# fabianschenk/REVO

Hardware: AMD Instinct MI355X
Metric: tracked frames/sec at 640x480, 4-level pyramid; ATE vs reference (higher is better)
Workload: dtype f32

## Files before the change

### revo_amd/csrc/revo_dev.h

```cpp
#pragma once
#include <hip/hip_runtime.h>
#include <stdint.h>
#include "../../include/revo_hip.h"

#define REVO_L REVO_MAX_LEVELS

struct LevelGeom {
  int w, h;
  int npix;
  float fx, fy, cx, cy;
  int patch;
  int hist_w, hist_h;
  int nchunk;
  int chunk_rows;
  int wpr;
  int nms_block_base;
  int has_orig;
  int pix_base;
  int edt_rows;
  int edt_block_base;
  int strip_base;
  int cc_base;
  int band_rows, nbands, band_base;
};

struct PyrGeom {
  int frame0;
  int fstride;
  int n_levels;
  int total_nms_blocks, total_pix, total_edt_blocks, total_strips, total_cc;
  int total_bands, any_banded;
  int hyst_force;
  int hyst_heavy_runs;
  int total_tiles;
  int pts_staged;
  float depth_min, depth_max;
  int canny_low, canny_high;
  int use_edge_hist;
  float n_percentage;
  double fill_thr[REVO_L];
  LevelGeom lv[REVO_L];
};

struct FramePlanes {
  uint8_t* gray[REVO_L];
  float* depth[REVO_L];
  uint2* cs[REVO_L];
  uint8_t* edges[REVO_L];
  uint8_t* edges_orig[REVO_L];
  int* scratch[REVO_L];
  float4* pts[REVO_L];
  float4* pts_trk[REVO_L];
  float* dt[REVO_L];
  float4* table[REVO_L];
  uint8_t* hist[REVO_L];
  int* chunk[REVO_L];
  unsigned* cmask[REVO_L];
  uint8_t* vb[REVO_L];
  int* npts;
  int* hist_nz;
  int* strip_tot;
  uint32_t* ebits[REVO_L];
  int* need_full;
  int* hyst_heavy;
  int* tile_base;
  float* stage[REVO_L];
  unsigned short* epre[REVO_L];
  int* stage_base;
};

struct PairDesc {
  const float4* pts[REVO_L];
  const int* npts;
  const float* dt[REVO_L];
  float R[9];
  float T[3];
};

struct TrackParams {
  int pyr_min_lvl, pyr_max_lvl;
  int lvl_begin, lvl_end;
  int check_init;
  int eval_only;
  int kspec[REVO_L];
  int redundant_n;
  float lambda_success_fac, lambda_fail_fac;
  float lambda_initial[REVO_L], step_size_min[REVO_L], convergence_eps[REVO_L];
  int max_its[REVO_L];
  float edge_distance[REVO_L];
  float huber_edge;
  int use_edge_filter;
  struct { float fx, fy, cx, cy; int w, h; } cam[REVO_L];
  int exact_sums;
};

struct EvalOut {
  float A[36];
  float b[6];
  float error;
  float mean_err;
  float sum_w, sum_u;
  int good, bad;
};

#define REVO_MAX_WIDTH 2048
#define NMS_ROWS 6
#define EDT_ROW_PX 1280
#ifndef REVO_HYST_LDS_MAX
#define REVO_HYST_LDS_MAX 158720
#endif
#ifndef TRACK_THREADS
#define TRACK_THREADS 512
#endif
#ifndef TRACK_MAX_CLUSTER
#define TRACK_MAX_CLUSTER 32
#endif
#define TRACK_KMAX 4
#define TRACK_NVAL 48
#define TRACK_NVAL_X 132
#define TRACK_MAIL_NVAL TRACK_NVAL_X

void launch_gray_depth(const PyrGeom& g, const FramePlanes& p, const uint8_t* d_bgr, const float* d_depth_f32,
                       const uint16_t* d_depth_u16, float u16_alpha, int B, hipStream_t s);
void launch_pyrdown(const PyrGeom& g, const FramePlanes& p, int lvl, int B, hipStream_t s, int parts = 3, bool stage_edges = false);
void launch_edge_prefix(const PyrGeom& g, const FramePlanes& p, int B, hipStream_t s);
void launch_canny_nms(const PyrGeom& g, const FramePlanes& p, int B, hipStream_t s);
void launch_hyst(const PyrGeom& g, const FramePlanes& p, int B, hipStream_t s);
void launch_fill(const PyrGeom& g, const FramePlanes& p, int B, hipStream_t s);
void launch_compact(const PyrGeom& g, const FramePlanes& p, int B, hipStream_t s);
void launch_tile_points(const PyrGeom& g, const FramePlanes& p, int B, hipStream_t s, int which = 3);
void launch_pyrdown_bgr(const uint8_t* src, int w, int h, uint8_t* dst, hipStream_t s);
void launch_colored_pcl(const PyrGeom& g, const FramePlanes& p, int frame, int lvl, int dense, const uint8_t* bgr_lvl,
                        int* chunk, unsigned* cmask, int* total, int cap, float* out8, hipStream_t s);
void launch_keyframe(const PyrGeom& g, const FramePlanes& p, int f0, int fstride, int count, hipStream_t s, int which = 3);
int launch_track(const PairDesc* d_descs, const TrackParams& prm, revo_pair_result* d_out, EvalOut* d_eval,
                 int n_pairs, unsigned long long* d_mail, unsigned* epoch_io, int cluster, unsigned* d_resident, hipStream_t s);
void launch_track_gate(unsigned* d_resident, unsigned want, hipStream_t s);
int launch_track_one(const PairDesc& desc, const TrackParams& prm, revo_pair_result* out, EvalOut* eval_out,
                     unsigned long long* d_mail, unsigned* epoch_io, int cluster, unsigned* seq_ptr, unsigned seq_val,
                     unsigned* d_resident, hipStream_t s);
void launch_solve6(const float* d_Ab , int n, float* d_x , hipStream_t s);
int track_blocks_per_cu();
void launch_grad_table(const PyrGeom& g, const FramePlanes& p, int f0, int fstride, int count, hipStream_t s);
struct VoteArgs { float RT[3][12]; const float4* pts[3]; const int* n[3]; };
void launch_vote(const PyrGeom& g, const FramePlanes& curr, int curr_frame, int lvl, int n_clouds, const VoteArgs& va,
                 int* d_marks , int* d_hist8 , unsigned* d_done ,
                 int* h_out8 , unsigned seq_val, int use_orig_edges,
                 hipStream_t s);
void launch_copy_cloud(float4* dst, const float4* src, int* dst_n, const int* src_n, hipStream_t s);
struct VoteDesc {
  float RT[3][12]; const float4* pts[3]; const int* n[3]; int n_clouds;
  const uint8_t* edges; const float* depth;
  int* marks; int* hist8; unsigned* done;
  int* host_out;
};
struct CloudCopyDesc { float4* dst; const float4* src; int* dst_n; const int* src_n; };
struct CopySeg { const void* src; void* dst; size_t bytes; };
void launch_vote_multi(const PyrGeom& g, int lvl, int n, const VoteDesc* d_descs, unsigned seq_val, hipStream_t s);
void launch_copy_cloud_multi(int n, const CloudCopyDesc* d_descs, hipStream_t s);
void launch_copy_segments(int n, const CopySeg* d_segs, hipStream_t s);

#define INFO_THREADS 256
#define INFO_CHUNK 1024
#define INFO_MAX_GROUPS 32
#define INFO_PART_DOUBLES 64
struct InfoParams {
  float fx, fy, cx, cy;
  int w, h;
  float edge_distance, huber_edge;
  int use_edge_filter, level;
};
static inline int info_groups(int npix) {
  const int g = (npix + 8 * INFO_CHUNK - 1) / (8 * INFO_CHUNK);
  return g < 1 ? 1 : (g > INFO_MAX_GROUPS ? INFO_MAX_GROUPS : g);
}
void launch_pair_info(const PairDesc* d_descs, const void* d_pose, int pose_stride, int flag_word, const InfoParams& prm,
                      int n_pairs, double* d_part, int* d_cnt, unsigned* d_ticket, revo_pair_info* d_out, hipStream_t s);
```

### revo_amd/csrc/revo_pyramid.hip

```cpp
#include "revo_dev.h"
#include "revo_nms_px.h"
#include <type_traits>

namespace {

#ifdef REVO_BUILD_PRIO
#define BUILD_PRIO() __builtin_amdgcn_s_setprio(REVO_BUILD_PRIO)
#else
#define BUILD_PRIO()
#endif

__device__ __forceinline__ int level_of(const PyrGeom& g, int v, int LevelGeom::*base) {
  int l = 0;
#pragma unroll
  for (int k = 1; k < REVO_L; ++k)
    if (k < g.n_levels && v >= g.lv[k].*base) l = k;
  return l;
}
__device__ __forceinline__ int clampi(int v, int lo, int hi) { return v < lo ? lo : (v > hi ? hi : v); }
__device__ __forceinline__ int reflect101(int i, int n) {
  if (i < 0) i = -i;
  if (i >= n) i = 2 * n - 2 - i;
  return i;
}

__device__ __forceinline__ uint32_t gray4(uint32_t a, uint32_t b, uint32_t c) {
  const int B0 = a & 255, G0 = (a >> 8) & 255, R0 = (a >> 16) & 255, B1 = a >> 24;
  const int G1 = b & 255, R1 = (b >> 8) & 255, B2 = (b >> 16) & 255, G2 = b >> 24;
  const int R2 = c & 255, B3 = (c >> 8) & 255, G3 = (c >> 16) & 255, R3 = c >> 24;
  const uint32_t y0 = (uint32_t)(B0 * 1868 + G0 * 9617 + R0 * 4899 + 8192) >> 14;
  const uint32_t y1 = (uint32_t)(B1 * 1868 + G1 * 9617 + R1 * 4899 + 8192) >> 14;
  const uint32_t y2 = (uint32_t)(B2 * 1868 + G2 * 9617 + R2 * 4899 + 8192) >> 14;
  const uint32_t y3 = (uint32_t)(B3 * 1868 + G3 * 9617 + R3 * 4899 + 8192) >> 14;
  return y0 | (y1 << 8) | (y2 << 16) | (y3 << 24);
}
__global__ void __launch_bounds__(256) k_gray_depth(const uint8_t* __restrict__ bgr, const float* __restrict__ depth_f32,
                                                    const uint16_t* __restrict__ depth_u16, float alpha,
                                                    uint8_t* __restrict__ gray, float* __restrict__ depth_out, int npix, int frame0) {
  BUILD_PRIO();
  const int f = frame0 + blockIdx.z;
  const int g16 = blockIdx.x * 256 + threadIdx.x;
  if (g16 * 16 >= npix) return;
  const uint4* src = reinterpret_cast<const uint4*>(bgr + (size_t)f * npix * 3) + (size_t)g16 * 3;
  const uint4 p = src[0], q = src[1], r = src[2];
  reinterpret_cast<uint4*>(gray + (size_t)f * npix)[g16] =
      make_uint4(gray4(p.x, p.y, p.z), gray4(p.w, q.x, q.y), gray4(q.z, q.w, r.x), gray4(r.y, r.z, r.w));
  if (depth_out == depth_f32) return;
  float4* dst = reinterpret_cast<float4*>(depth_out + (size_t)f * npix) + (size_t)g16 * 4;
  if (depth_u16) {
    const uint4* raw = reinterpret_cast<const uint4*>(depth_u16 + (size_t)f * npix) + (size_t)g16 * 2;
    const uint4 u = raw[0], v = raw[1];
    const uint32_t wds[8] = {u.x, u.y, u.z, u.w, v.x, v.y, v.z, v.w};
#pragma unroll
    for (int k = 0; k < 4; ++k) {
      float4 d;
      d.x = (float)(wds[2 * k] & 0xffff) * alpha + 0.0f;
      d.y = (float)(wds[2 * k] >> 16) * alpha + 0.0f;
      d.z = (float)(wds[2 * k + 1] & 0xffff) * alpha + 0.0f;
      d.w = (float)(wds[2 * k + 1] >> 16) * alpha + 0.0f;
      dst[k] = d;
    }
  } else {
    const float4* in = reinterpret_cast<const float4*>(depth_f32 + (size_t)f * npix) + (size_t)g16 * 4;
    const float4 d0 = in[0], d1 = in[1], d2 = in[2], d3 = in[3];
    dst[0] = d0; dst[1] = d1; dst[2] = d2; dst[3] = d3;
  }
}

struct EdgeStage {
  const uint2* cs;
  const unsigned short* epre;
  const int* base;
  float* out;
  int wpr, tiles_total;
};
template <bool GRAY, bool DEPTH, bool STAGE = false>
__global__ void __launch_bounds__(256) k_pyrdown(const uint8_t* __restrict__ src, int sw, int sh, uint8_t* __restrict__ dst,
                                                 int dw, int dh, const float* __restrict__ dsrc, float* __restrict__ ddst, int frame0,
                                                 int fstride, uint8_t* __restrict__ vsrc, float dmin, float dmax, EdgeStage es) {
  BUILD_PRIO();
  static_assert(!STAGE || DEPTH, "staging rides on the depth half");
  const int f = frame0 + fstride * blockIdx.z;
  src += (size_t)f * sw * sh;
  dst += (size_t)f * dw * dh;
  dsrc += (size_t)f * sw * sh;
  ddst += (size_t)f * dw * dh;
  vsrc += (size_t)f * (sw >> 3) * sh;
  const int gw = dw >> 2, gh = (dh + 1) >> 1;
  const int i = blockIdx.x * 256 + threadIdx.x;
  if (i >= gw * gh) return;
  const int gx = i % gw, gy = i / gw;
  const int oy = 2 * gy;
  const int nrows = (oy + 1 < dh) ? 2 : 1;
  const int swords = sw >> 2;
  const uint32_t* srcw = reinterpret_cast<const uint32_t*>(src);
  const int w1i = 2 * gx;
  int hs[7][4];
#pragma unroll
  for (int r = 0; r < 7; ++r) {
    if (GRAY && r < 2 * nrows + 3) {
      const uint32_t* row = srcw + (size_t)reflect101(2 * oy - 2 + r, sh) * swords;
      uint32_t w0 = row[max(w1i - 1, 0)];
      const uint32_t w1 = row[w1i], w2 = row[w1i + 1];
      uint32_t w3 = row[min(w1i + 2, swords - 1)];
      if (gx == 0) w0 = (((w1 >> 16) & 0xffu) << 16) | (((w1 >> 8) & 0xffu) << 24);
      if (gx == gw - 1) w3 = (w2 >> 16) & 0xffu;
      const int b[11] = {(int)((w0 >> 16) & 0xffu), (int)(w0 >> 24),
                         (int)(w1 & 0xffu), (int)((w1 >> 8) & 0xffu), (int)((w1 >> 16) & 0xffu), (int)(w1 >> 24),
                         (int)(w2 & 0xffu), (int)((w2 >> 8) & 0xffu), (int)((w2 >> 16) & 0xffu), (int)(w2 >> 24),
                         (int)(w3 & 0xffu)};
#pragma unroll
      for (int j = 0; j < 4; ++j) hs[r][j] = b[2 * j] + b[2 * j + 4] + 4 * (b[2 * j + 1] + b[2 * j + 3]) + 6 * b[2 * j + 2];
    } else {
#pragma unroll
      for (int j = 0; j < 4; ++j) hs[r][j] = 0;
    }
  }
#pragma unroll
  for (int q = 0; q < 2; ++q) {
    if (q >= nrows) break;
    if (GRAY) {
      uint32_t packed = 0;
#pragma unroll
      for (int j = 0; j < 4; ++j) {
        const int v = hs[2 * q][j] + hs[2 * q + 4][j] + 4 * (hs[2 * q + 1][j] + hs[2 * q + 3][j]) + 6 * hs[2 * q + 2][j];
        packed |= (uint32_t)((v + 128) >> 8) << (8 * j);
      }
      reinterpret_cast<uint32_t*>(dst + (size_t)(oy + q) * dw)[gx] = packed;
    }
    if (!DEPTH) continue;
    const float* d0 = dsrc + (size_t)(2 * (oy + q)) * sw + 8 * gx;
    const float4 a0 = *reinterpret_cast<const float4*>(d0), a1 = *reinterpret_cast<const float4*>(d0 + 4);
    const float4 c0 = *reinterpret_cast<const float4*>(d0 + sw), c1 = *reinterpret_cast<const float4*>(d0 + sw + 4);
    const float top[8] = {a0.x, a0.y, a0.z, a0.w, a1.x, a1.y, a1.z, a1.w};
    const float bot[8] = {c0.x, c0.y, c0.z, c0.w, c1.x, c1.y, c1.z, c1.w};
    unsigned vt = 0, vbm = 0;
#pragma unroll
    for (int k = 0; k < 8; ++k) {
      vt |= (isfinite(top[k]) && top[k] > dmin && top[k] < dmax) ? 1u << k : 0u;
      vbm |= (isfinite(bot[k]) && bot[k] > dmin && bot[k] < dmax) ? 1u << k : 0u;
    }
    vsrc[(size_t)(2 * (oy + q)) * (sw >> 3) + gx] = (uint8_t)vt;
    vsrc[(size_t)(2 * (oy + q) + 1) * (sw >> 3) + gx] = (uint8_t)vbm;
    if (STAGE) {
      const int wc = (8 * gx) >> 5, sh8 = (8 * gx) & 31;
#pragma unroll
      for (int rr = 0; rr < 2; ++rr) {
        const int y = 2 * (oy + q) + rr;
        const uint32_t E = es.cs[((size_t)f * sh + y) * es.wpr + wc].y;
        uint32_t eb = (E >> sh8) & 0xffu;
        if (eb) {
          const int tile = (y >> 5) * es.wpr + wc;
          int pos = es.base[(size_t)f * es.tiles_total + tile] + (int)es.epre[((size_t)f * sh + y) * es.wpr + wc] +
                    __popc(E & ((1u << sh8) - 1u));
// ... 1385 lines not shown
  const uint32_t E = y < h ? csw[(size_t)y * wpr + wc].y : 0u;
  uint32_t v = (has_vb && y < h) ? tile_valid_word(g, pl, l, f, y, wc, E) : E;
  if (!has_vb)
    for (uint32_t m = v; m; m &= m - 1) {
      const int b = __ffs(m) - 1;
      if (!depth_ok(depth[(size_t)y * w + x0 + b], g.depth_min, g.depth_max)) v &= ~(1u << b);
    }
  const int cnt = __popc(v);
  int incl = cnt;
#pragma unroll
  for (int o = 1; o < 32; o <<= 1) {
    const int u = __shfl_up(incl, o, 32);
    if (r >= o) incl += u;
  }
  const int total = __shfl(incl, 31, 32);
  if (total == 0) return;
  unsigned short* src = s_src[threadIdx.x >> 5];
  const bool staged = STAGED && has_vb;
  unsigned short* esrc = s_esrc[STAGED ? (threadIdx.x >> 5) : 0];
  {
    int o = incl - cnt;
    int ebase = 0;
    if (staged) {
      const int ec = __popc(E);
      int ei = ec;
#pragma unroll
      for (int q = 1; q < 32; q <<= 1) {
        const int u = __shfl_up(ei, q, 32);
        if (r >= q) ei += u;
      }
      ebase = ei - ec;
    }
    for (uint32_t m = v; m; m &= m - 1, ++o) {
      const int b = __ffs(m) - 1;
      src[o] = (unsigned short)((r << 5) | b);
      if (staged) esrc[o] = (unsigned short)(ebase + __popc(E & ((1u << b) - 1u)));
    }
  }
  float4* out = pl.pts_trk[l] + (size_t)f * lv.npix + tile_first;
  const float* stage_t = staged ? pl.stage[l] + (size_t)f * lv.npix + pl.stage_base[(size_t)f * g.total_tiles + tg] : nullptr;
  for (int k0 = r; k0 < total; k0 += 4 * 32) {
    int rb[4];
    float Z[4];
#pragma unroll
    for (int q = 0; q < 4; ++q) rb[q] = k0 + 32 * q < total ? (int)src[k0 + 32 * q] : -1;
    if (staged) {
#pragma unroll
      for (int q = 0; q < 4; ++q) Z[q] = rb[q] >= 0 ? stage_t[esrc[k0 + 32 * q]] : 0.0f;
    } else {
#pragma unroll
      for (int q = 0; q < 4; ++q) Z[q] = rb[q] >= 0 ? depth[(size_t)(y0 + (rb[q] >> 5)) * w + x0 + (rb[q] & 31)] : 0.0f;
    }
#pragma unroll
    for (int q = 0; q < 4; ++q) {
      if (rb[q] < 0) continue;
      const float X = __fdiv_rn(Z[q] * ((float)(x0 + (rb[q] & 31)) - lv.cx), lv.fx);
      const float Y = __fdiv_rn(Z[q] * ((float)(y0 + (rb[q] >> 5)) - lv.cy), lv.fy);
      out[k0 + 32 * q] = make_float4(X, Y, Z[q], 1.0f);
    }
  }
}

__device__ __forceinline__ int block_exclusive_scan(int* a, int n, int* s_part) {
  const int tid = threadIdx.x, lane = tid & 63, wave = tid >> 6;
  const int per = (n + 1023) / 1024;
  const int b = min(n, tid * per), e = min(n, b + per);
  int sum = 0;
  for (int i = b; i < e; ++i) sum += a[i];
  int incl = sum;
#pragma unroll
  for (int o = 1; o < 64; o <<= 1) {
    const int v = __shfl_up(incl, o);
    if (lane >= o) incl += v;
  }
  if (lane == 63) s_part[wave] = incl;
  __syncthreads();
  int run = incl - sum, total = 0;
#pragma unroll
  for (int k = 0; k < 16; ++k) {
    const int wv = s_part[k];
    run += k < wave ? wv : 0;
    total += wv;
  }
  for (int i = b; i < e; ++i) { const int c = a[i]; a[i] = run; run += c; }
  return total;
}


__global__ void __launch_bounds__(256) k_pyrdown_bgr(const uint8_t* __restrict__ src, int w, int h,
                                                     uint8_t* __restrict__ dst) {
  const int dw = w >> 1, dh = h >> 1;
  const int i = blockIdx.x * 256 + threadIdx.x;
  if (i >= dw * dh) return;
  const int x = i % dw, y = i / dw;
  const int kk[5] = {1, 4, 6, 4, 1};
  int acc[3] = {0, 0, 0};
#pragma unroll
  for (int j = 0; j < 5; ++j) {
    const uint8_t* row = src + (size_t)reflect101(2 * y + j - 2, h) * w * 3;
    int rs[3] = {0, 0, 0};
#pragma unroll
    for (int t = 0; t < 5; ++t) {
      const uint8_t* px = row + (size_t)reflect101(2 * x + t - 2, w) * 3;
      rs[0] += kk[t] * px[0]; rs[1] += kk[t] * px[1]; rs[2] += kk[t] * px[2];
    }
    acc[0] += kk[j] * rs[0]; acc[1] += kk[j] * rs[1]; acc[2] += kk[j] * rs[2];
  }
  uint8_t* o = dst + (size_t)i * 3;
  o[0] = (uint8_t)((acc[0] + 128) >> 8); o[1] = (uint8_t)((acc[1] + 128) >> 8); o[2] = (uint8_t)((acc[2] + 128) >> 8);
}

template <bool WRITE>
__global__ void __launch_bounds__(256) k_pcl_walk(LevelGeom lv, float dmin, float dmax, const float* __restrict__ depth,
                                                  const uint8_t* __restrict__ edges, const uint8_t* __restrict__ bgr,
                                                  int dense, int* __restrict__ chunk, unsigned* __restrict__ cmask,
                                                  const int* __restrict__ total, int cap, float4* __restrict__ out) {
  const int i = blockIdx.x * 256 + threadIdx.x;
  if (i >= lv.w * lv.nchunk) return;
  const int x = i % lv.w, c = i / lv.w;
  const int yb = c * lv.chunk_rows, ye = min(lv.h, yb + lv.chunk_rows);
  const size_t slot = (size_t)x * lv.nchunk + c;
  if (!WRITE) {
    unsigned vm = 0;
    for (int y = yb; y < ye; ++y) {
      const size_t p = (size_t)y * lv.w + x;
      if ((dense || edges[p]) && depth_ok(depth[p], dmin, dmax)) vm |= 1u << (y - yb);
    }
    cmask[slot] = vm;
    chunk[slot] = __popc(vm);
  } else {
    if (*total > cap) return;
    int o = chunk[slot];
    for (unsigned m = cmask[slot]; m; m &= m - 1) {
      const int y = yb + __ffs(m) - 1;
      const size_t p = (size_t)y * lv.w + x;
      const float Z = depth[p];
      const float X = __fdiv_rn(Z * ((float)x - lv.cx), lv.fx);
      const float Y = __fdiv_rn(Z * ((float)y - lv.cy), lv.fy);
      const uint8_t* px = bgr + p * 3;
      out[2 * o] = make_float4(X, Y, Z, 1.0f);
      out[2 * o + 1] = make_float4(__fdiv_rn((float)px[2], 255.0f), __fdiv_rn((float)px[1], 255.0f),
                                   __fdiv_rn((float)px[0], 255.0f), 1.0f);
      ++o;
    }
  }
}

__global__ void __launch_bounds__(1024) k_pcl_scan(int* chunk, int n, int* total) {
  __shared__ int s_part[1024];
  const int t = block_exclusive_scan(chunk, n, s_part);
  if (threadIdx.x == 0) *total = t;
}

#define EDT_INF (1 << 29)
#define EDT_THREADS 1024
#define EDT_COL_GROUPS(h) ((h) > 1024 ? 64 : ((h) > 512 ? 32 : 16))
__global__ void __launch_bounds__(EDT_THREADS) k_edt_cols(PyrGeom g, FramePlanes pl, int f0, int fstride, int nframes) {
  __shared__ int s_first[EDT_THREADS];
  __shared__ int s_last[EDT_THREADS];
  const int f = f0 + (blockIdx.x % nframes) * fstride;
  int l = 0, sidx = blockIdx.x / nframes, ngroups = 16, ncols = 64;
  for (int k = 0; k < g.n_levels; ++k) {
    ngroups = EDT_COL_GROUPS(g.lv[k].h);
    ncols = EDT_THREADS / ngroups;
    const int ns = (g.lv[k].w + ncols - 1) / ncols;
    if (sidx < ns) { l = k; break; }
    sidx -= ns;
  }
  const LevelGeom& lv = g.lv[l];
  const int col = threadIdx.x % ncols, grp = threadIdx.x / ncols;
  const int x = sidx * ncols + col;
  const int rpg = (lv.h + ngroups - 1) / ngroups;
  const int yb = min(lv.h, grp * rpg), ye = min(lv.h, yb + rpg);
  const bool in = x < lv.w;
  const uint8_t* edges = pl.edges[l] + (size_t)f * lv.npix;
  unsigned em = 0;
  if ((lv.w & 31) == 0 && (ncols & 31) == 0) {
    const uint2* csw = pl.cs[l] + (size_t)f * lv.h * lv.wpr;
    const int r = threadIdx.x & 31;
    const int wc = (sidx * ncols + (col & ~31)) >> 5;
    uint32_t v = 0;
    if (yb + r < ye && wc < lv.wpr) v = csw[(size_t)(yb + r) * lv.wpr + wc].y;
    em = tile_transpose32(v, r);
    if (!in) em = 0;
  } else if (in) {
#pragma unroll 8
    for (int y = yb; y < ye; ++y) em |= (edges[(size_t)y * lv.w + x] ? 1u : 0u) << (y - yb);
  }
  s_first[grp * ncols + col] = em ? yb + __ffs(em) - 1 : EDT_INF;
  s_last[grp * ncols + col] = em ? yb + 31 - __clz(em) : -EDT_INF;
  __syncthreads();
  if (!in) return;
  int above = -EDT_INF, below = EDT_INF;
  for (int k = 0; k < grp; ++k) above = max(above, s_last[k * ncols + col]);
  for (int k = ngroups - 1; k > grp; --k) below = min(below, s_first[k * ncols + col]);
  uint16_t* gd = reinterpret_cast<uint16_t*>(pl.scratch[l]) + (size_t)f * lv.npix;
  const int FAR = 1 << 20;
  int du = (above <= -EDT_INF) ? FAR : (yb - above);
  const int dbelow = (below >= EDT_INF) ? FAR : (below - yb);
  for (int y = yb; y < ye; ++y) {
    const int k = y - yb;
    const unsigned hi = em >> k;
    du = (hi & 1u) ? 0 : du;
    const int dn = hi ? __ffs(hi) - 1 : dbelow - k;
    const int m = min(du, dn);
    gd[(size_t)y * lv.w + x] = (uint16_t)(m >= 0xffff ? 0xffff : m);
    du += 1;
  }
}

__device__ __forceinline__ float sqrt_rn_int(float x) {
  const float s = __builtin_amdgcn_sqrtf(x);
  const unsigned si = __float_as_uint(s);
  const float sd = __uint_as_float(si - 1u), su = __uint_as_float(si + 1u);
  const float rd = __builtin_fmaf(-sd, s, x), ru = __builtin_fmaf(-su, s, x);
  float r = (rd <= 0.0f) ? sd : s;
  r = (ru > 0.0f) ? su : r;
  return r;
}
__global__ void __launch_bounds__(256) k_edt_rows(PyrGeom g, FramePlanes pl, int f0, int fstride) {
  extern __shared__ int s_g2[];
  const int f = f0 + blockIdx.z * fstride;
  const int l = level_of(g, blockIdx.x, &LevelGeom::edt_block_base);
  const LevelGeom lv = g.lv[l];
  const int w = lv.w;
  const int y0 = (blockIdx.x - lv.edt_block_base) * lv.edt_rows;
  const int nr = min(lv.edt_rows, lv.h - y0);
  const int pad = w + 4, pitch = w + 2 * pad;
  const uint16_t* gd = reinterpret_cast<const uint16_t*>(pl.scratch[l]) + (size_t)f * lv.npix + (size_t)y0 * w;
  const int4 inf4 = make_int4(EDT_INF, EDT_INF, EDT_INF, EDT_INF);
  const int padq = pad >> 2, wq = w >> 2;
  for (int r = 0; r < nr; ++r) {
    int4* row4 = reinterpret_cast<int4*>(s_g2 + r * pitch);
    for (int i = threadIdx.x; i < padq; i += 256) { row4[i] = inf4; row4[padq + wq + i] = inf4; }
    const uint2* src = reinterpret_cast<const uint2*>(gd + r * w);
    for (int i = threadIdx.x; i < wq; i += 256) {
      const uint2 q = src[i];
      const int d0 = (int)(q.x & 0xffffu), d1 = (int)(q.x >> 16), d2 = (int)(q.y & 0xffffu), d3 = (int)(q.y >> 16);
      row4[padq + i] = make_int4(d0 == 0xffff ? EDT_INF : __mul24(d0, d0), d1 == 0xffff ? EDT_INF : __mul24(d1, d1),
                                 d2 == 0xffff ? EDT_INF : __mul24(d2, d2), d3 == 0xffff ? EDT_INF : __mul24(d3, d3));
    }
  }
  __syncthreads();
  float* dt = pl.dt[l] + (size_t)f * lv.npix + (size_t)y0 * w;
  const int dq = 256 / w, dr = 256 - dq * w;
  int r = threadIdx.x / w, x = threadIdx.x - r * w;
  for (int p = threadIdx.x; p < nr * w; p += 256) {
    const int* c = s_g2 + r * pitch + pad + x;
    int best = c[0];
    for (int d = 1; d < w && d * d < best; d += 4) {
      int m = best;
#pragma unroll
      for (int j = 0; j < 4; ++j) {
        const int dj = d + j;
        m = min(m, dj * dj + min(c[-dj], c[dj]));
      }
      best = m;
    }
    dt[p] = best >= EDT_INF ? sqrtf(1e15f) : sqrt_rn_int((float)best);
    x += dr; r += dq;
    if (x >= w) { x -= w; ++r; }
  }
}

__global__ void __launch_bounds__(256) k_grad_table(PyrGeom g, FramePlanes pl, int f0, int fstride) {
  const int f = f0 + blockIdx.z * fstride;
  const int l = blockIdx.y;
  const LevelGeom& lv = g.lv[l];
  const int i = blockIdx.x * 256 + threadIdx.x;
  if (i >= lv.npix) return;
  const float* dt = pl.dt[l] + (size_t)f * lv.npix;
  float4 o = make_float4(0.f, 0.f, 0.f, 0.f);
  if (i >= lv.w && i < lv.w * (lv.h - 1)) {
    o.x = 0.5f * (dt[i - 1] - dt[i + 1]);
    o.y = 0.5f * (dt[i - lv.w] - dt[i + lv.w]);
    o.z = dt[i];
  }
  pl.table[l][(size_t)f * lv.npix + i] = o;
}

__global__ void __launch_bounds__(256) k_vote_mark(VoteArgs a, float fx, float fy, float cx, float cy, int W, int H,
                                                   int* marks) {
  const int c = blockIdx.y;
  const int n = *a.n[c];
  const float* R = a.RT[c];
  const float* T = R + 9;
  const float4* pts = a.pts[c];
  for (int i = blockIdx.x * 256 + threadIdx.x; i < n; i += gridDim.x * 256) {
    const float4 p = pts[i];
    float q[3];
#pragma unroll
    for (int r = 0; r < 3; ++r) q[r] = ((R[r] * p.x + R[3 + r] * p.y) + R[6 + r] * p.z) + T[r];
    const float u = __fdiv_rn(fx * q[0], q[2]) + cx;
    const float v = __fdiv_rn(fy * q[1], q[2]) + cy;
    if (u >= 0 && u < (float)W && v >= 0 && v < (float)H)
      atomicOr(&marks[(int)floorf(v) * W + (int)floorf(u)], 1 << c);
  }
}

__global__ void __launch_bounds__(256) k_vote_hist(int* marks, const uint8_t* edges, const float* depth, int npix,
                                                   float dmin, float dmax, int* hist8, unsigned* done, int* host_out,
                                                   unsigned seq_val) {
  __shared__ int s_h[8];
  __shared__ bool s_last;
  if (threadIdx.x < 8) s_h[threadIdx.x] = 0;
  __syncthreads();
  for (int i = blockIdx.x * 256 + threadIdx.x; i < npix; i += gridDim.x * 256) {
    const int m = marks[i];
    if (m) marks[i] = 0;
    const float Z = depth[i];
    if (depth_ok(Z, dmin, dmax)) {
      const int val = __popc(m);
      atomicAdd(&s_h[val], 1);
      if (edges[i] > 0) atomicAdd(&s_h[4 + val], 1);
    }
  }
  __syncthreads();
  if (threadIdx.x < 8 && s_h[threadIdx.x]) atomicAdd(&hist8[threadIdx.x], s_h[threadIdx.x]);
  __threadfence();
  __syncthreads();
  if (threadIdx.x == 0) s_last = (atomicAdd(done, 1u) == gridDim.x - 1);
  __syncthreads();
  if (s_last) {
    if (threadIdx.x < 8) host_out[threadIdx.x] = atomicExch(&hist8[threadIdx.x], 0);
    if (threadIdx.x == 0) *done = 0u;
    __threadfence_system();
    __syncthreads();
    if (threadIdx.x == 0) *(volatile int*)&host_out[8] = (int)seq_val;
  }
}

__global__ void __launch_bounds__(256) k_copy_cloud(float4* __restrict__ dst, const float4* __restrict__ src,
                                                    int* __restrict__ dst_n, const int* __restrict__ src_n) {
  const int n = *src_n;
  for (int i = blockIdx.x * 256 + threadIdx.x; i < n; i += gridDim.x * 256) dst[i] = src[i];
  if (blockIdx.x == 0 && threadIdx.x == 0) *dst_n = n;
}

__global__ void __launch_bounds__(256) k_vote_mark_multi(const VoteDesc* __restrict__ descs, float fx, float fy, float cx,
                                                         float cy, int W, int H) {
  const VoteDesc& d = descs[blockIdx.z];
  const int c = blockIdx.y;
  if (c >= d.n_clouds) return;
  const int n = *d.n[c];
  const float* R = d.RT[c];
  const float* T = R + 9;
  const float4* pts = d.pts[c];
  int* marks = d.marks;
  for (int i = blockIdx.x * 256 + threadIdx.x; i < n; i += gridDim.x * 256) {
    const float4 p = pts[i];
    float q[3];
#pragma unroll
    for (int r = 0; r < 3; ++r) q[r] = ((R[r] * p.x + R[3 + r] * p.y) + R[6 + r] * p.z) + T[r];
    const float u = __fdiv_rn(fx * q[0], q[2]) + cx;
    const float v = __fdiv_rn(fy * q[1], q[2]) + cy;
    if (u >= 0 && u < (float)W && v >= 0 && v < (float)H)
      atomicOr(&marks[(int)floorf(v) * W + (int)floorf(u)], 1 << c);
  }
}

__global__ void __launch_bounds__(256) k_vote_hist_multi(const VoteDesc* __restrict__ descs, int npix, float dmin, float dmax,
                                                         unsigned seq_val) {
  const VoteDesc& d = descs[blockIdx.y];
  int* marks = d.marks;
  __shared__ int s_h[8];
  __shared__ bool s_last;
  if (threadIdx.x < 8) s_h[threadIdx.x] = 0;
  __syncthreads();
  for (int i = blockIdx.x * 256 + threadIdx.x; i < npix; i += gridDim.x * 256) {
    const int m = marks[i];
    if (m) marks[i] = 0;
    const float Z = d.depth[i];
    if (depth_ok(Z, dmin, dmax)) {
      const int val = __popc(m);
      atomicAdd(&s_h[val], 1);
      if (d.edges[i] > 0) atomicAdd(&s_h[4 + val], 1);
    }
  }
  __syncthreads();
  if (threadIdx.x < 8 && s_h[threadIdx.x]) atomicAdd(&d.hist8[threadIdx.x], s_h[threadIdx.x]);
  __threadfence();
  __syncthreads();
  if (threadIdx.x == 0) s_last = (atomicAdd(d.done, 1u) == gridDim.x - 1);
  __syncthreads();
  if (s_last) {
    if (threadIdx.x < 8) d.host_out[threadIdx.x] = atomicExch(&d.hist8[threadIdx.x], 0);
    if (threadIdx.x == 0) *d.done = 0u;
    __threadfence_system();
    __syncthreads();
    if (threadIdx.x == 0) *(volatile int*)&d.host_out[8] = (int)seq_val;
  }
}

__global__ void __launch_bounds__(256) k_copy_cloud_multi(const CloudCopyDesc* __restrict__ descs) {
  const CloudCopyDesc& d = descs[blockIdx.y];
  const int n = *d.src_n;
  for (int i = blockIdx.x * 256 + threadIdx.x; i < n; i += gridDim.x * 256) d.dst[i] = d.src[i];
  if (blockIdx.x == 0 && threadIdx.x == 0) *d.dst_n = n;
}

__global__ void __launch_bounds__(256) k_copy_segments(const CopySeg* __restrict__ segs) {
  const CopySeg& sg = segs[blockIdx.y];
  const char* src = (const char*)sg.src;
  char* dst = (char*)sg.dst;
  const size_t bytes = sg.bytes;
  const size_t step = (size_t)gridDim.x * 256;
  if ((((uintptr_t)src | (uintptr_t)dst | bytes) & 15) == 0) {
    const uint4* s4 = (const uint4*)src;
    uint4* d4 = (uint4*)dst;
    for (size_t i = blockIdx.x * 256 + threadIdx.x; i < bytes / 16; i += step) d4[i] = s4[i];
  } else {
    for (size_t i = blockIdx.x * 256 + threadIdx.x; i < bytes; i += step) dst[i] = src[i];
  }
}
// ... 7 lines not shown
  hipLaunchKernelGGL(k_gray_depth, grid, dim3(256), 0, s, d_bgr, d_depth_f32, d_depth_u16, u16_alpha, p.gray[0],
                     p.depth[0], npix, g.frame0);
}

void launch_pyrdown(const PyrGeom& g, const FramePlanes& p, int lvl, int B, hipStream_t s, int parts, bool stage_edges) {
  const LevelGeom& d = g.lv[lvl];
  const LevelGeom& sl = g.lv[lvl - 1];
  dim3 grid(((d.w / 4) * ((d.h + 1) / 2) + 255) / 256, 1, B);
  EdgeStage es{};
  if (stage_edges) {
    int tb = 0;
    for (int k = 0; k < lvl - 1; ++k) tb += g.lv[k].wpr * g.lv[k].nchunk;
    es.cs = p.cs[lvl - 1]; es.epre = p.epre[lvl - 1]; es.base = p.stage_base + tb; es.out = p.stage[lvl - 1];
    es.wpr = sl.wpr; es.tiles_total = g.total_tiles;
  }
#define PYRDOWN_ARGS p.gray[lvl - 1], sl.w, sl.h, p.gray[lvl], d.w, d.h, p.depth[lvl - 1], p.depth[lvl], g.frame0, g.fstride, p.vb[lvl - 1], g.depth_min, g.depth_max, es
  if (parts == 1) hipLaunchKernelGGL((k_pyrdown<true, false>), grid, dim3(256), 0, s, PYRDOWN_ARGS);
  else if (parts == 2 && stage_edges) hipLaunchKernelGGL((k_pyrdown<false, true, true>), grid, dim3(256), 0, s, PYRDOWN_ARGS);
  else if (parts == 2) hipLaunchKernelGGL((k_pyrdown<false, true>), grid, dim3(256), 0, s, PYRDOWN_ARGS);
  else hipLaunchKernelGGL((k_pyrdown<true, true>), grid, dim3(256), 0, s, PYRDOWN_ARGS);
#undef PYRDOWN_ARGS
}

void launch_edge_prefix(const PyrGeom& g, const FramePlanes& p, int B, hipStream_t s) {
  if (g.n_levels < 2) return;
  hipLaunchKernelGGL(k_edge_prefix, dim3((g.n_levels - 1) * B), dim3(1024), 0, s, g, p);
}

void launch_canny_nms(const PyrGeom& g, const FramePlanes& p, int B, hipStream_t s) {
  hipLaunchKernelGGL(k_canny_nms4, dim3(g.total_nms_blocks, 1, B), dim3(256), 0, s, g, p);
}

void launch_hyst(const PyrGeom& g, const FramePlanes& p, int B, hipStream_t s) {
  size_t e_bytes = 0, ec_bytes = 0;
  for (int l = 0; l < g.n_levels; ++l) {
    const size_t nw = (size_t)g.lv[l].h * g.lv[l].wpr;
    const size_t e = ((size_t)(g.lv[l].h + 2) * g.lv[l].wpr + 2) * 4, c = (nw + (nw + 2) / 2) * 4;
    e_bytes = e > e_bytes ? e : e_bytes;
    ec_bytes = e + c > ec_bytes ? e + c : ec_bytes;
  }
  static bool attr_set = false;
  if (!attr_set) {
    (void)hipFuncSetAttribute(reinterpret_cast<const void*>(k_hyst<true>), hipFuncAttributeMaxDynamicSharedMemorySize, REVO_HYST_LDS_MAX);
    (void)hipFuncSetAttribute(reinterpret_cast<const void*>(k_hyst<false>), hipFuncAttributeMaxDynamicSharedMemorySize, REVO_HYST_LDS_MAX);
    attr_set = true;
  }
  const int force = g.hyst_force;
  const bool fits_single = ec_bytes + 4096 <= REVO_HYST_LDS_MAX;
  const bool banded = force >= 0 ? force == 1 : !fits_single;
  const int only_flagged = banded && g.total_bands > 0 ? 1 : 0;
  if (only_flagged) {
    static bool attr2 = false;
    if (!attr2) {
      (void)hipFuncSetAttribute(reinterpret_cast<const void*>(k_hyst_band), hipFuncAttributeMaxDynamicSharedMemorySize, HB_LDS_WORDS * 4);
      (void)hipFuncSetAttribute(reinterpret_cast<const void*>(k_hyst_out), hipFuncAttributeMaxDynamicSharedMemorySize, HB_LDS_WORDS * 4);
      (void)hipFuncSetAttribute(reinterpret_cast<const void*>(k_hyst_seam), hipFuncAttributeMaxDynamicSharedMemorySize, 64 * 1024);
      (void)hipGetLastError();
      attr2 = true;
    }
    size_t seam_lds = 4, out_lds = 4;
    for (int l = 0; l < g.n_levels; ++l) {
      const LevelGeom& lv = g.lv[l];
      const size_t nwb = (size_t)lv.band_rows * lv.wpr;
      out_lds = std::max(out_lds, nwb * 4);
      if (lv.nbands > 1) seam_lds = std::max(seam_lds, (size_t)lv.nbands * (size_t)(HB_LDS_WORDS / 2 / 32 + 64) * 4);
    }
    hipLaunchKernelGGL(k_hyst_band, dim3(g.total_bands * B), dim3(HB_THREADS), HB_LDS_WORDS * 4, s, g, p);
    if (g.any_banded) hipLaunchKernelGGL(k_hyst_seam, dim3(g.n_levels * B), dim3(HS_THREADS), seam_lds, s, g, p, 0);
    hipLaunchKernelGGL(k_hyst_out, dim3(g.total_bands * B), dim3(HO_THREADS), out_lds, s, g, p, 0);
  }
  const bool mixed = !banded && fits_single && g.hyst_heavy_runs > 0 && g.total_bands > 0 && g.lv[0].nbands > 1;
  if (mixed) {
    static bool attr3 = false;
    if (!attr3) {
      (void)hipFuncSetAttribute(reinterpret_cast<const void*>(k_hyst_mixed), hipFuncAttributeMaxDynamicSharedMemorySize, REVO_HYST_LDS_MAX);
      (void)hipFuncSetAttribute(reinterpret_cast<const void*>(k_hyst_out), hipFuncAttributeMaxDynamicSharedMemorySize, HB_LDS_WORDS * 4);
      (void)hipFuncSetAttribute(reinterpret_cast<const void*>(k_hyst_seam), hipFuncAttributeMaxDynamicSharedMemorySize, 64 * 1024);
      (void)hipGetLastError();
      attr3 = true;
    }
    const LevelGeom& l0 = g.lv[0];
    const size_t seam_lds = std::max<size_t>(4, (size_t)l0.nbands * (size_t)(HB_LDS_WORDS / 2 / 32 + 64) * 4);
    const size_t out_lds = std::max<size_t>(4, (size_t)l0.band_rows * l0.wpr * 4);
    hipLaunchKernelGGL(k_hyst_mixed, dim3((l0.nbands + g.n_levels) * B), dim3(HYST_THREADS), REVO_HYST_LDS_MAX, s, g, p, B);
    hipLaunchKernelGGL(k_hyst_seam, dim3(B), dim3(HS_THREADS), seam_lds, s, g, p, 1);
    hipLaunchKernelGGL(k_hyst_out, dim3(l0.nbands * B), dim3(HO_THREADS), out_lds, s, g, p, 1);
    hipLaunchKernelGGL(k_hyst<true>, dim3(std::min(32, g.n_levels * B)), dim3(HYST_THREADS), REVO_HYST_LDS_MAX, s, g, p, 1, B);
    return;
  }
  const int n_wg = only_flagged ? std::min(32, g.n_levels * B) : g.n_levels * B;
  if (ec_bytes + 4096 <= REVO_HYST_LDS_MAX)
    hipLaunchKernelGGL(k_hyst<true>, dim3(n_wg), dim3(HYST_THREADS), REVO_HYST_LDS_MAX, s, g, p, only_flagged, B);
  else if (e_bytes <= REVO_HYST_LDS_MAX)
    hipLaunchKernelGGL(k_hyst<false>, dim3(n_wg), dim3(HYST_THREADS), e_bytes, s, g, p, only_flagged, B);
  else
    hipLaunchKernelGGL((k_hyst<false, true>), dim3(n_wg), dim3(HYST_THREADS), 16, s, g, p, only_flagged, B);
}

void launch_fill(const PyrGeom& g, const FramePlanes& p, int B, hipStream_t s) {
  bool any = false;
  for (int l = 1; l < g.n_levels; ++l) any = any || g.lv[l].has_orig;
  if (!any) return;
  if (g.lv[0].npix <= 640 * 480) {
    hipLaunchKernelGGL(k_fill, dim3(1, 1, B), dim3(1024), 0, s, g, p, 0);
    return;
  }
  for (int l = 1; l < g.n_levels; ++l) {
    if (!g.lv[l].has_orig) continue;
    const int n = (g.lv[l - 1].w / 2) * (g.lv[l - 1].h / 2);
    hipLaunchKernelGGL(k_fill, dim3(std::min(64, (n + 1023) / 1024), 1, B), dim3(1024), 0, s, g, p, l);
  }
}

void launch_tile_points(const PyrGeom& g, const FramePlanes& p, int B, hipStream_t s, int which) {
  if (which & 1) hipLaunchKernelGGL(k_tile_count, dim3(g.n_levels * B), dim3(1024), 0, s, g, p);
  const int groups = (g.total_tiles + PT_TILES - 1) / PT_TILES;
  if ((which & 2) && g.pts_staged) hipLaunchKernelGGL(k_pts_tiles<true>, dim3(groups * B), dim3(32 * PT_TILES), 0, s, g, p);
  else if (which & 2) hipLaunchKernelGGL(k_pts_tiles<false>, dim3(groups * B), dim3(32 * PT_TILES), 0, s, g, p);
}

void launch_compact(const PyrGeom& g, const FramePlanes& p, int B, hipStream_t s) {
  dim3 grid(g.total_strips * B);
  hipLaunchKernelGGL(k_compact_walk<false>, grid, dim3(CW_COLS * CW_LANES_COUNT), 0, s, g, p);
  hipLaunchKernelGGL(k_compact_walk<true>, grid, dim3(CW_COLS * CW_LANES), 0, s, g, p);
}

void launch_pyrdown_bgr(const uint8_t* src, int w, int h, uint8_t* dst, hipStream_t s) {
  hipLaunchKernelGGL(k_pyrdown_bgr, dim3(((w / 2) * (h / 2) + 255) / 256), dim3(256), 0, s, src, w, h, dst);
}

void launch_colored_pcl(const PyrGeom& g, const FramePlanes& p, int frame, int lvl, int dense, const uint8_t* bgr_lvl,
                        int* chunk, unsigned* cmask, int* total, int cap, float* out8, hipStream_t s) {
  const LevelGeom& lv = g.lv[lvl];
  const float* depth = p.depth[lvl] + (size_t)frame * lv.npix;
  const uint8_t* edges = p.edges[lvl] + (size_t)frame * lv.npix;
  const int n = lv.w * lv.nchunk;
  dim3 grid((n + 255) / 256);
  hipLaunchKernelGGL(k_pcl_walk<false>, grid, dim3(256), 0, s, lv, g.depth_min, g.depth_max, depth, edges, bgr_lvl, dense,
                     chunk, cmask, total, cap, (float4*)out8);
  hipLaunchKernelGGL(k_pcl_scan, dim3(1), dim3(1024), 0, s, chunk, n, total);
  hipLaunchKernelGGL(k_pcl_walk<true>, grid, dim3(256), 0, s, lv, g.depth_min, g.depth_max, depth, edges, bgr_lvl, dense,
                     chunk, cmask, total, cap, (float4*)out8);
}

void launch_keyframe(const PyrGeom& g, const FramePlanes& p, int f0, int fstride, int count, hipStream_t s, int which) {
  int strips = 0;
  for (int l = 0; l < g.n_levels; ++l) {
    const int ncols = EDT_THREADS / EDT_COL_GROUPS(g.lv[l].h);
    strips += (g.lv[l].w + ncols - 1) / ncols;
  }
  if (which & 1) hipLaunchKernelGGL(k_edt_cols, dim3(strips * count), dim3(EDT_THREADS), 0, s, g, p, f0, fstride, count);
  size_t rows_lds = 0;
  for (int l = 0; l < g.n_levels; ++l) rows_lds = std::max(rows_lds, (size_t)g.lv[l].edt_rows * (3 * g.lv[l].w + 8) * sizeof(int));
  if (which & 2) hipLaunchKernelGGL(k_edt_rows, dim3(g.total_edt_blocks, 1, count), dim3(256), rows_lds, s, g, p, f0, fstride);
}

void launch_grad_table(const PyrGeom& g, const FramePlanes& p, int f0, int fstride, int count, hipStream_t s) {
  hipLaunchKernelGGL(k_grad_table, dim3((g.lv[0].npix + 255) / 256, g.n_levels, count), dim3(256), 0, s, g, p, f0, fstride);
}

void launch_vote(const PyrGeom& g, const FramePlanes& curr, int curr_frame, int lvl, int n_clouds, const VoteArgs& va,
                 int* d_marks, int* d_hist8, unsigned* d_done, int* h_out8, unsigned seq_val, int use_orig_edges, hipStream_t s) {
  const LevelGeom& lv = g.lv[lvl];
  if (n_clouds > 0)
    hipLaunchKernelGGL(k_vote_mark, dim3(32, n_clouds), dim3(256), 0, s, va, lv.fx, lv.fy, lv.cx, lv.cy, lv.w, lv.h, d_marks);
  const uint8_t* edges = (use_orig_edges ? curr.edges_orig[lvl] : curr.edges[lvl]) + (size_t)curr_frame * lv.npix;
  hipLaunchKernelGGL(k_vote_hist, dim3(16), dim3(256), 0, s, d_marks, edges,
                     curr.depth[lvl] + (size_t)curr_frame * lv.npix, lv.npix, g.depth_min, g.depth_max, d_hist8, d_done, h_out8,
                     seq_val);
}

void launch_copy_cloud(float4* dst, const float4* src, int* dst_n, const int* src_n, hipStream_t s) {
  hipLaunchKernelGGL(k_copy_cloud, dim3(16), dim3(256), 0, s, dst, src, dst_n, src_n);
}

void launch_vote_multi(const PyrGeom& g, int lvl, int n, const VoteDesc* d_descs, unsigned seq_val, hipStream_t s) {
  const LevelGeom& lv = g.lv[lvl];
  hipLaunchKernelGGL(k_vote_mark_multi, dim3(32, 3, n), dim3(256), 0, s, d_descs, lv.fx, lv.fy, lv.cx, lv.cy, lv.w, lv.h);
  hipLaunchKernelGGL(k_vote_hist_multi, dim3(16, n), dim3(256), 0, s, d_descs, lv.npix, g.depth_min, g.depth_max, seq_val);
}

void launch_copy_cloud_multi(int n, const CloudCopyDesc* d_descs, hipStream_t s) {
  hipLaunchKernelGGL(k_copy_cloud_multi, dim3(16, n), dim3(256), 0, s, d_descs);
}

void launch_copy_segments(int n, const CopySeg* d_segs, hipStream_t s) {
  hipLaunchKernelGGL(k_copy_segments, dim3(64, n), dim3(256), 0, s, d_segs);
}
```

Measured before the change: 119,000.

## Vectorize EDT row pass: four pixels per thread with register-reused quad loads

Rewrites the row pass of the distance transform so each thread handles four adjacent pixels. It loads int4 quads from LDS and reuses them across neighbouring offsets in a rolling register window, then writes float4 results. The LDS fill is flattened into one loop over all rows with padding writes, and the block size becomes EDT_ROW_PX/4 threads. This aims to cut LDS load count and loop overhead per pixel. The cost is early termination per group of four pixels, so each thread searches until the slowest of the four converges.

Result: faster. 120,900, median of 6 (+1.6%).

```diff
diff --git a/revo_amd/csrc/revo_dev.h b/revo_amd/csrc/revo_dev.h
--- a/revo_amd/csrc/revo_dev.h
+++ b/revo_amd/csrc/revo_dev.h
@@ -106,6 +106,7 @@
 #define REVO_MAX_WIDTH 2048
 #define NMS_ROWS 6
 #define EDT_ROW_PX 1280
+#define EDT_ROW_THREADS (EDT_ROW_PX / 4)
 #ifndef REVO_HYST_LDS_MAX
 #define REVO_HYST_LDS_MAX 158720
 #endif
diff --git a/revo_amd/csrc/revo_edt_px.h b/revo_amd/csrc/revo_edt_px.h
--- /dev/null
+++ b/revo_amd/csrc/revo_edt_px.h
@@ -0,0 +1,99 @@
+#pragma once
+#include <math.h>
+#include <stdint.h>
+
+#if defined(__HIPCC__) || defined(__CUDACC__)
+#define EDT_HD __host__ __device__ __forceinline__
+#define EDT_UNROLL _Pragma("unroll")
+#else
+#define EDT_HD inline
+#define EDT_UNROLL
+#endif
+
+#define EDT_INF (1 << 29)
+
+#if defined(__HIP_DEVICE_COMPILE__)
+typedef int edt_quad __attribute__((ext_vector_type(4)));
+EDT_HD void edt_keep(edt_quad& q) { asm volatile("" : "+v"(q)); }
+#else
+struct alignas(16) edt_quad {
+  int v[4];
+  int operator[](int i) const { return v[i]; }
+};
+EDT_HD void edt_keep(edt_quad&) {}
+#endif
+
+EDT_HD int edt_min(int a, int b) { return a < b ? a : b; }
+EDT_HD int edt_max(int a, int b) { return a > b ? a : b; }
+
+EDT_HD int edt_g2(int d16) { return d16 == 0xffff ? EDT_INF : d16 * d16; }
+
+template <bool FIRST>
+EDT_HD void edt_trip(int t, const edt_quad* pr, const edt_quad* pl, const edt_quad& in_r, edt_quad& out_r, edt_quad& out_l,
+                     const edt_quad& in_l, int best[4]) {
+  out_r = *pr;
+  out_l = *pl;
+  edt_keep(out_r);
+  edt_keep(out_l);
+  const int R[8] = {in_r[0], in_r[1], in_r[2], in_r[3], out_r[0], out_r[1], out_r[2], out_r[3]};
+  const int L[8] = {out_l[0], out_l[1], out_l[2], out_l[3], in_l[0], in_l[1], in_l[2], in_l[3]};
+  const int d0 = 4 * t;
+  int dd[4];
+EDT_UNROLL
+  for (int j = 0; j < 4; ++j) dd[j] = (d0 + j) * (d0 + j);
+EDT_UNROLL
+  for (int i = 0; i < 4; ++i) {
+    int m[4];
+EDT_UNROLL
+    for (int j = 0; j < 4; ++j) m[j] = edt_min(R[i + j], L[4 + i - j]) + dd[j];
+    if (!FIRST) best[i] = edt_min(edt_min(best[i], m[0]), m[1]);
+    else best[i] = edt_min(best[i], m[1]);
+    best[i] = edt_min(edt_min(best[i], m[2]), m[3]);
+  }
+}
+
+EDT_HD bool edt_more(int t, int w, const int best[4]) {
+  const int d0 = 4 * t;
+  return d0 < w && d0 * d0 < edt_max(edt_max(best[0], best[1]), edt_max(best[2], best[3]));
+}
+
+EDT_HD void edt_search4(const int* row, int q, int w, int best[4]) {
+  const edt_quad* c = reinterpret_cast<const edt_quad*>(row) + q;
+  edt_quad A = c[0], B, O, I;
+  edt_keep(A);
+EDT_UNROLL
+  for (int i = 0; i < 4; ++i) best[i] = A[i];
+  edt_trip<true>(0, c + 1, c - 1, A, B, O, A, best);
+  for (int t = 1;; t += 2) {
+    if (!edt_more(t, w, best)) break;
+    edt_trip<false>(t, c + t + 1, c - t - 1, B, A, I, O, best);
+    if (!edt_more(t + 1, w, best)) break;
+    edt_trip<false>(t + 1, c + t + 2, c - t - 2, A, B, O, I, best);
+  }
+}
+
+EDT_HD float edt_sqrt_fix(float x, float s) {
+  uint32_t si;
+  __builtin_memcpy(&si, &s, 4);
+  const uint32_t di = si - 1u, ui = si + 1u;
+  float sd, su;
+  __builtin_memcpy(&sd, &di, 4);
+  __builtin_memcpy(&su, &ui, 4);
+  const float rd = __builtin_fmaf(-sd, s, x), ru = __builtin_fmaf(-su, s, x);
+  float r = (rd <= 0.0f) ? sd : s;
+  r = (ru > 0.0f) ? su : r;
+  return r;
+}
+EDT_HD float edt_sqrt_rn_int(float x) {
+#if defined(__HIP_DEVICE_COMPILE__)
+  return edt_sqrt_fix(x, __builtin_amdgcn_sqrtf(x));
+#else
+  return edt_sqrt_fix(x, sqrtf(x));
+#endif
+}
+EDT_HD float edt_dt(int best) {
+  const float r = edt_sqrt_rn_int((float)best);
+  return best >= EDT_INF ? sqrtf(1e15f) : r;
+}
+
+EDT_HD int edt_div_small(int a, float inv) { return (int)(((float)a + 0.5f) * inv); }
diff --git a/revo_amd/csrc/revo_pyramid.hip b/revo_amd/csrc/revo_pyramid.hip
--- a/revo_amd/csrc/revo_pyramid.hip
+++ b/revo_amd/csrc/revo_pyramid.hip
@@ -1,5 +1,6 @@
 #include "revo_dev.h"
 #include "revo_nms_px.h"
+#include "revo_edt_px.h"
 #include <type_traits>
 
 namespace {
@@ -1691,7 +1692,6 @@
   if (threadIdx.x == 0) *total = t;
 }
 
-#define EDT_INF (1 << 29)
 #define EDT_THREADS 1024
 #define EDT_COL_GROUPS(h) ((h) > 1024 ? 64 : ((h) > 512 ? 32 : 16))
 __global__ void __launch_bounds__(EDT_THREADS) k_edt_cols(PyrGeom g, FramePlanes pl, int f0, int fstride, int nframes) {
@@ -1748,17 +1748,8 @@
   }
 }
 
-__device__ __forceinline__ float sqrt_rn_int(float x) {
-  const float s = __builtin_amdgcn_sqrtf(x);
-  const unsigned si = __float_as_uint(s);
-  const float sd = __uint_as_float(si - 1u), su = __uint_as_float(si + 1u);
-  const float rd = __builtin_fmaf(-sd, s, x), ru = __builtin_fmaf(-su, s, x);
-  float r = (rd <= 0.0f) ? sd : s;
-  r = (ru > 0.0f) ? su : r;
-  return r;
-}
-__global__ void __launch_bounds__(256) k_edt_rows(PyrGeom g, FramePlanes pl, int f0, int fstride) {
-  extern __shared__ int s_g2[];
+__global__ void __launch_bounds__(EDT_ROW_THREADS) k_edt_rows(PyrGeom g, FramePlanes pl, int f0, int fstride) {
+  extern __shared__ __attribute__((aligned(16))) int s_g2[];
   const int f = f0 + blockIdx.z * fstride;
   const int l = level_of(g, blockIdx.x, &LevelGeom::edt_block_base);
   const LevelGeom lv = g.lv[l];
@@ -1766,39 +1757,28 @@
   const int y0 = (blockIdx.x - lv.edt_block_base) * lv.edt_rows;
   const int nr = min(lv.edt_rows, lv.h - y0);
   const int pad = w + 4, pitch = w + 2 * pad;
-  const uint16_t* gd = reinterpret_cast<const uint16_t*>(pl.scratch[l]) + (size_t)f * lv.npix + (size_t)y0 * w;
+  const uint2* src = reinterpret_cast<const uint2*>(reinterpret_cast<const uint16_t*>(pl.scratch[l]) + (size_t)f * lv.npix + (size_t)y0 * w);
   const int4 inf4 = make_int4(EDT_INF, EDT_INF, EDT_INF, EDT_INF);
-  const int padq = pad >> 2, wq = w >> 2;
-  for (int r = 0; r < nr; ++r) {
-    int4* row4 = reinterpret_cast<int4*>(s_g2 + r * pitch);
-    for (int i = threadIdx.x; i < padq; i += 256) { row4[i] = inf4; row4[padq + wq + i] = inf4; }
-    const uint2* src = reinterpret_cast<const uint2*>(gd + r * w);
-    for (int i = threadIdx.x; i < wq; i += 256) {
-      const uint2 q = src[i];
-      const int d0 = (int)(q.x & 0xffffu), d1 = (int)(q.x >> 16), d2 = (int)(q.y & 0xffffu), d3 = (int)(q.y >> 16);
-      row4[padq + i] = make_int4(d0 == 0xffff ? EDT_INF : __mul24(d0, d0), d1 == 0xffff ? EDT_INF : __mul24(d1, d1),
-                                 d2 == 0xffff ? EDT_INF : __mul24(d2, d2), d3 == 0xffff ? EDT_INF : __mul24(d3, d3));
-    }
-  }
-  __syncthreads();
-  float* dt = pl.dt[l] + (size_t)f * lv.npix + (size_t)y0 * w;
-  const int dq = 256 / w, dr = 256 - dq * w;
-  int r = threadIdx.x / w, x = threadIdx.x - r * w;
-  for (int p = threadIdx.x; p < nr * w; p += 256) {
-    const int* c = s_g2 + r * pitch + pad + x;
-    int best = c[0];
-    for (int d = 1; d < w && d * d < best; d += 4) {
-      int m = best;
-#pragma unroll
-      for (int j = 0; j < 4; ++j) {
-        const int dj = d + j;
-        m = min(m, dj * dj + min(c[-dj], c[dj]));
-      }
-      best = m;
-    }
-    dt[p] = best >= EDT_INF ? sqrtf(1e15f) : sqrt_rn_int((float)best);
-    x += dr; r += dq;
-    if (x >= w) { x -= w; ++r; }
+  const int padq = pad >> 2, wq = w >> 2, pitchq = pitch >> 2;
+  int4* lds4 = reinterpret_cast<int4*>(s_g2);
+  const float inv_wq = __builtin_amdgcn_rcpf((float)wq);
+  for (int j = threadIdx.x; j < nr * wq; j += EDT_ROW_THREADS) {
+    const uint2 q = src[j];
+    const int r = edt_div_small(j, inv_wq), i = j - __mul24(r, wq);
+    int4* row4 = lds4 + __mul24(r, pitchq);
+    row4[i] = inf4;
+    row4[padq + wq + i] = inf4;
+    row4[padq + i] = make_int4(edt_g2((int)(q.x & 0xffffu)), edt_g2((int)(q.x >> 16)), edt_g2((int)(q.y & 0xffffu)), edt_g2((int)(q.y >> 16)));
+  }
+  for (int j = threadIdx.x; j < 2 * nr; j += EDT_ROW_THREADS) lds4[__mul24(j >> 1, pitchq) + ((j & 1) ? padq + 2 * wq : wq)] = inf4;
+  __syncthreads();
+  float4* dt4 = reinterpret_cast<float4*>(pl.dt[l] + (size_t)f * lv.npix + (size_t)y0 * w);
+  const float inv = __builtin_amdgcn_rcpf((float)nr);
+  for (int i = threadIdx.x; i < nr * wq; i += EDT_ROW_THREADS) {
+    const int q = edt_div_small(i, inv), r = i - __mul24(q, nr);
+    int best[4];
+    edt_search4(s_g2 + __mul24(r, pitch) + pad, q, w, best);
+    dt4[__mul24(r, wq) + q] = make_float4(edt_dt(best[0]), edt_dt(best[1]), edt_dt(best[2]), edt_dt(best[3]));
   }
 }
 
@@ -2112,7 +2092,7 @@
   if (which & 1) hipLaunchKernelGGL(k_edt_cols, dim3(strips * count), dim3(EDT_THREADS), 0, s, g, p, f0, fstride, count);
   size_t rows_lds = 0;
   for (int l = 0; l < g.n_levels; ++l) rows_lds = std::max(rows_lds, (size_t)g.lv[l].edt_rows * (3 * g.lv[l].w + 8) * sizeof(int));
-  if (which & 2) hipLaunchKernelGGL(k_edt_rows, dim3(g.total_edt_blocks, 1, count), dim3(256), rows_lds, s, g, p, f0, fstride);
+  if (which & 2) hipLaunchKernelGGL(k_edt_rows, dim3(g.total_edt_blocks, 1, count), dim3(EDT_ROW_THREADS), rows_lds, s, g, p, f0, fstride);
 }
 
 void launch_grad_table(const PyrGeom& g, const FramePlanes& p, int f0, int fstride, int count, hipStream_t s) {
```
